# a-ludi/dentist

Hardware: AMD Instinct MI355X
Metric: gap-bases closed/sec (higher is better)
Workload: dtype u8

## Files before the change

### dentist_amd/csrc/dh_tjoin.h

```cpp
#ifndef DH_TJOIN_H
#define DH_TJOIN_H
#include <stdint.h>

#if defined(__HIPCC__)
#define TJ_HD __host__ __device__ __forceinline__
#else
#define TJ_HD inline
#endif

#define TJ_SLOT_BITS 14
#define TJ_SLOTS (1 << TJ_SLOT_BITS)
#define TJ_CAP 8192
#define TJ_THREADS 1024
#define TJ_RUN (TJ_THREADS / 64)
#define TJ_QBATCH 4
#define TJ_MAXK 16
#define TJ_EMPTY (~0ull)

#define DH_ST_TJ_HITCAP 0x80
#define DH_ST_TJ_OVERFLOW 0x100

TJ_HD uint32_t tj_home(uint32_t canon) { return (canon * 0x9E3779B1u) >> (32 - TJ_SLOT_BITS); }
TJ_HD uint64_t tj_slot(uint32_t canon, uint32_t ori, uint32_t idx) { return ((uint64_t)canon << 32) | (ori << 31) | idx; }

template <class Claim>
TJ_HD void tj_insert(uint64_t *tab, uint64_t v, Claim claim)
{
    uint32_t h = tj_home((uint32_t)(v >> 32));
    while (!claim(tab + h, v)) h = (h + 1) & (TJ_SLOTS - 1);
}

template <class F>
TJ_HD void tj_walk(const uint64_t *tab, uint32_t canon, F f)
{
    for (uint32_t h = tj_home(canon);; h = (h + 1) & (TJ_SLOTS - 1)) {
        const uint64_t s = tab[h];
        if (s == TJ_EMPTY) return;
        if ((uint32_t)(s >> 32) == canon) f((uint32_t)s);
    }
}

struct TjMatch {
    int32_t fwd, rev;
    uint32_t emit;
};
TJ_HD TjMatch tj_match(const uint64_t *tab, uint32_t canon, uint32_t bori, bool pal, int32_t tcap, int32_t strands)
{
    int32_t runf = 0, runr = 0;
    tj_walk(tab, canon, [&](uint32_t lo) {
        const bool same = (lo >> 31) == bori;
        runf += (same || pal) ? 1 : 0;
        runr += (!same || pal) ? 1 : 0;
    });
    TjMatch m;
    m.emit = ((runf > 0 && runf <= tcap && (strands & 1)) ? 1u : 0u) | ((runr > 0 && runr <= tcap && (strands & 2)) ? 2u : 0u);
    m.fwd = (m.emit & 1u) ? runf : 0;
    m.rev = (m.emit & 2u) ? runr : 0;
    return m;
}

#ifndef DH_TJOIN_SLOT_CODE_ONLY
#include "dh_device.h"
#include "dh_join.h"

struct TjView {
    const uint32_t *gent;
    int32_t ngroups;
    const int4 *units;
    int32_t nunits;
    int32_t read0;
    uint64_t *segtab;
    uint64_t *hits;
    int64_t hits_cap;
    unsigned long long *cursor;
    uint32_t *queue;
    int32_t *status;
};

extern "C" {
void dhk_tj_group_offsets(hipStream_t st, const uint32_t *dir, int32_t ngroups, int32_t k, int32_t shift, int64_t nb,
                          uint32_t *gent);
void dhk_tjoin(hipStream_t st, DbView B, IndexView ix, DhOpts o, TjView t, int32_t ncu);
}
#endif
#endif
```

### dentist_amd/csrc/dh_tjoin.hip

```cpp
#include <hip/hip_runtime.h>
#include <stdint.h>
#include <stdio.h>
#include <stdlib.h>

#include <algorithm>

#include "dh_kmer.h"
#include "dh_tjoin.h"

#define LANES 64
#define HIT_QBITS 24

#ifdef DH_TJ_PROF
__device__ unsigned long long g_tj_prof[4];
#define TP(i) if (tid == 0) { const unsigned long long t_ = wall_clock64(); atomicAdd(&g_tj_prof[i], t_ - tp_); tp_ = t_; }
#define TP_BEGIN unsigned long long tp_ = wall_clock64();
extern "C" void dhk_tj_prof_dump()
{
    unsigned long long h[4];
    (void)hipMemcpyFromSymbol(h, HIP_SYMBOL(g_tj_prof), sizeof(h));
    if (h[3])
        fprintf(stderr, "[tj prof] k_tjoin, %llu units: table build %.1f roll + probe %.1f write %.1f us per unit and block\n", h[3],
                h[0] / 100.0 / h[3], h[1] / 100.0 / h[3], h[2] / 100.0 / h[3]);
    unsigned long long z[4] = {0};
    (void)hipMemcpyToSymbol(HIP_SYMBOL(g_tj_prof), z, sizeof(z));
}
#else
#define TP(i)
#define TP_BEGIN
#endif

__global__ void __launch_bounds__(256)
k_tj_group_offsets(const uint32_t *__restrict__ dir, int32_t ngroups, int32_t k, int32_t shift, int64_t nb, uint32_t *__restrict__ gent)
{
    const int32_t g = blockIdx.x * blockDim.x + threadIdx.x;
    if (g > ngroups) return;
    int64_t b = (int64_t)(((uint64_t)g << (2 * k)) >> shift);
    b = b < nb ? b : nb;
    gent[g] = dir[b - 1];
}

static __device__ __forceinline__ uint32_t tj_pack8(uint64_t w)
{
    uint64_t x = __builtin_bswap64(w) & 0x0303030303030303ull;
    x = (x | (x >> 6)) & 0x000F000F000F000Full;
    x = (x | (x >> 12)) & 0x000000FF000000FFull;
    return (uint32_t)((x | (x >> 24)) & 0xFFFFull);
}

template <bool WRITE>
static __device__ uint32_t tj_read(const DbView &B, const IndexView &ix, const DhOpts &o, const KmerSampler &smp, const uint64_t *tab,
                                   int32_t r, int lane, uint32_t g0, uint64_t *__restrict__ out, uint32_t limit, uint32_t *cur)
{
    constexpr int PER = 8, STEP = LANES * PER;
    constexpr uint64_t BAD = 0xFCFCFCFCFCFCFCFCull;
    const int64_t bo = B.off[r];
    const int32_t blen = (int32_t)(B.off[r + 1] - bo);
    const uint8_t *b = B.bases + bo;
    const int k = o.k;
    const int32_t npos = blen - k + 1;
    const uint32_t kmask = k >= 16 ? 0xFFFFFFFFu : ((1u << (2 * k)) - 1u);
    const uint32_t kbits = (1u << k) - 1u;
    uint32_t cnt = 0;
    uint64_t n0 = 0, n1 = 0, n2 = 0, nm = 0;
    auto fetch = [&](int32_t q0) {
        if (q0 < npos) {
            n0 = load8(b + q0);
            n1 = load8(b + q0 + 8);
            n2 = load8(b + q0 + 16);
            if (B.mask_bits) nm = load8(B.mask_bits + ((bo + q0) >> 3)) >> ((bo + q0) & 7);
        }
    };
    fetch(lane * PER);
    for (int32_t base = 0; base < npos; base += STEP) {
        const int32_t q0 = base + lane * PER;
        const uint64_t w0 = n0, w1 = n1, w2 = n2;
        const uint32_t mbits = (uint32_t)nm;
        fetch(q0 + STEP);
        if (q0 >= npos) continue;
        uint32_t nbits = 0;
        if ((w0 | w1 | w2) & BAD) {
            for (int i = 0; i < 8; i++) {
                nbits |= (((w0 >> (8 * i)) & 0xFC) ? 1u : 0u) << i;
                nbits |= (((w1 >> (8 * i)) & 0xFC) ? 1u : 0u) << (8 + i);
                nbits |= (((w2 >> (8 * i)) & 0xFC) ? 1u : 0u) << (16 + i);
            }
        }
        const uint64_t P = ((uint64_t)tj_pack8(w0) << 32) | ((uint64_t)tj_pack8(w1) << 16) | (uint64_t)tj_pack8(w2);
        uint64_t R = __brevll(~P);
        R = (((R >> 1) & 0x5555555555555555ull) | ((R & 0x5555555555555555ull) << 1)) >> 16;
#pragma unroll
        for (int j = 0; j < PER; j++) {
            const int32_t q = q0 + j;
            const uint32_t km = (uint32_t)(P >> (48 - 2 * k - 2 * j)) & kmask;
            const uint32_t rc = (uint32_t)(R >> (2 * j)) & kmask;
            const uint32_t canon = km < rc ? km : rc;
            const bool em = q < npos && !(((nbits | mbits) >> j) & kbits) && kmer_sampled((uint64_t)canon, smp);
            if (!em) continue;
            const uint32_t bori = km != canon ? 1u : 0u;
            const bool pal = km == rc;
            const TjMatch m = tj_match(tab, canon, bori, pal, o.tcap, o.strands);
            if (!WRITE)
                cnt += (uint32_t)(m.fwd + m.rev);
            else if (m.emit) {
                tj_walk(tab, canon, [&](uint32_t lo) {
                    const bool same = (lo >> 31) == bori;
                    const int64_t gv = (int64_t)(ix.ent[g0 + (lo & 0x7FFFFFFFu)].y & ((1ull << 40) - 1));
                    for (int32_t strand = 0; strand < 2; strand++) {
                        if (!(m.emit & (1u << strand)) || !(strand ? (!same || pal) : (same || pal))) continue;
                        const int32_t qs = strand ? blen - k - q : q;
                        const int64_t D = gv + ix.sepv - qs;
                        const uint32_t slot = atomicAdd(cur, 1u);
                        if (slot < limit) out[slot] = ((uint64_t)strand << 63) | ((uint64_t)D << HIT_QBITS) | (uint32_t)qs;
                        cnt++;
                    }
                });
            }
        }
    }
    return cnt;
}

__global__ void __launch_bounds__(TJ_THREADS, 1)
k_tjoin(DbView B, IndexView ix, DhOpts o, TjView t)
{
    __shared__ uint64_t tab[TJ_SLOTS];
    __shared__ uint32_t s_cnt[TJ_RUN], s_cur[TJ_RUN];
    __shared__ unsigned long long s_base;
    __shared__ int32_t s_work, s_ok;
    const int tid = threadIdx.x, lane = tid & (LANES - 1), wv = tid / LANES;
    const KmerSampler smp = kmer_sampler(o.kmer_mod, o.k);
    const uint64_t kmask = (1ull << (2 * o.k)) - 1;
    int32_t have = -1;
    uint32_t g0 = 0;
    TP_BEGIN
    for (;;) {
        __syncthreads();
        if (tid == 0) s_work = (int32_t)atomicAdd(t.queue, (uint32_t)TJ_QBATCH);
        __syncthreads();
        const int32_t u0 = s_work;
        if (u0 >= t.nunits) break;
#pragma unroll 1
        for (int32_t u = u0; u < min(u0 + TJ_QBATCH, t.nunits); u++) {
            const int4 un = t.units[u];
            if (un.x != have) {
                have = un.x;
                uint32_t g1 = 0;
                g0 = 0;
                if ((uint32_t)un.x < (uint32_t)t.ngroups) {
                    g0 = t.gent[un.x];
                    g1 = t.gent[un.x + 1];
                }
                if (g1 - g0 > (uint32_t)TJ_CAP || g1 > (uint32_t)ix.n || g1 < g0) {
                    if (tid == 0) atomicOr(t.status, DH_ST_TJ_OVERFLOW);
                    g1 = g0;
                }
                for (int32_t i = tid; i < TJ_SLOTS; i += TJ_THREADS) tab[i] = TJ_EMPTY;
                __syncthreads();
                for (uint32_t e = g0 + tid; e < g1; e += TJ_THREADS) {
                    const uint64_t x = ix.ent[e].x;
                    tj_insert(tab, tj_slot((uint32_t)(x & kmask), (uint32_t)(x >> 63), e - g0), [](uint64_t *p, uint64_t v) {
                        return atomicCAS((unsigned long long *)p, (unsigned long long)TJ_EMPTY, (unsigned long long)v) == TJ_EMPTY;
                    });
                }
                __syncthreads();
                TP(0)
            }
            const int32_t r = un.y + wv;
            const bool mine = r < un.z;
            uint32_t c = mine ? tj_read<false>(B, ix, o, smp, tab, r, lane, g0, nullptr, 0u, nullptr) : 0u;
            for (int off = LANES / 2; off > 0; off >>= 1) c += __shfl_xor(c, off, LANES);
            if (lane == 0) {
                s_cnt[wv] = c;
                s_cur[wv] = 0;
            }
            __syncthreads();
            if (tid == 0) {
                unsigned long long total = 0;
                for (int i = 0; i < TJ_RUN; i++) total += s_cnt[i];
                const unsigned long long base = total ? atomicAdd(t.cursor, total) : 0ull;
                const bool ok = base + total <= (unsigned long long)t.hits_cap;
                if (!ok) atomicOr(t.status, DH_ST_TJ_HITCAP);
                s_base = base;
                s_ok = ok ? 1 : 0;
            }
            __syncthreads();
            TP(1)
            if (mine && s_ok) {
                unsigned long long first = s_base;
                for (int i = 0; i < wv; i++) first += s_cnt[i];
                if (c >= (1u << 24) || first >= (1ull << 40)) {
                    if (lane == 0) atomicOr(t.status, DH_ST_TJ_OVERFLOW);
                } else {
                    if (c) tj_read<true>(B, ix, o, smp, tab, r, lane, g0, t.hits + first, c, &s_cur[wv]);
                    if (lane == 0) t.segtab[r - t.read0] = (first << 24) | c;
                }
            }
            __syncthreads();
            TP(2)
#ifdef DH_TJ_PROF
            if (tid == 0) atomicAdd(&g_tj_prof[3], 1ull);
#endif
        }
    }
}

extern "C" void dhk_tj_group_offsets(hipStream_t st, const uint32_t *dir, int32_t ngroups, int32_t k, int32_t shift, int64_t nb,
                                     uint32_t *gent)
{
    hipLaunchKernelGGL(k_tj_group_offsets, dim3((unsigned)((ngroups + 1 + 255) / 256)), dim3(256), 0, st, dir, ngroups, k, shift, nb, gent);
}

extern "C" void dhk_tjoin(hipStream_t st, DbView B, IndexView ix, DhOpts o, TjView t, int32_t ncu)
{
    if (t.nunits <= 0) return;
    const int32_t batches = (t.nunits + TJ_QBATCH - 1) / TJ_QBATCH;
    hipLaunchKernelGGL(k_tjoin, dim3((unsigned)std::min(batches, std::max(1, ncu))), dim3(TJ_THREADS), 0, st, B, ix, o, t);
#ifdef DH_TJ_PROF
    if (getenv("DH_TRACE")) {
        (void)hipStreamSynchronize(st);
        dhk_tj_prof_dump();
    }
#endif
}
```

Measured before the change: 2.515 million.

## Stash matching k-mer positions in LDS to skip full re-scan in write pass

During the count pass, each wave records in a per-wave LDS stash the read positions whose k-mer produced hits. The write pass then recomputes only those k-mers from two 8-byte loads and emits hits, instead of re-rolling and re-probing the whole read. Reads that are too long or overflow the stash fall back to the original full second pass, and an env var forces the old two-pass path. This adds LDS usage, which might stay within one-block-per-CU occupancy, plus an extra atomic per matching position during counting.

```diff
diff --git a/dentist_amd/csrc/dh_tjoin.h b/dentist_amd/csrc/dh_tjoin.h
--- a/dentist_amd/csrc/dh_tjoin.h
+++ b/dentist_amd/csrc/dh_tjoin.h
@@ -15,6 +15,8 @@
 #define TJ_RUN (TJ_THREADS / 64)
 #define TJ_QBATCH 4
 #define TJ_MAXK 16
+#define TJ_STASH 1008
+#define TJ_STASH_POSBITS 16
 #define TJ_EMPTY (~0ull)
 
 #define DH_ST_TJ_HITCAP 0x80
@@ -59,6 +61,44 @@
     return m;
 }
 
+TJ_HD uint32_t tj_pack8(uint64_t w)
+{
+    uint64_t x = __builtin_bswap64(w) & 0x0303030303030303ull;
+    x = (x | (x >> 6)) & 0x000F000F000F000Full;
+    x = (x | (x >> 12)) & 0x000000FF000000FFull;
+    return (uint32_t)((x | (x >> 24)) & 0xFFFFull);
+}
+
+TJ_HD uint32_t tj_brev32(uint32_t x)
+{
+#if defined(__HIP_DEVICE_COMPILE__)
+    return __brev(x);
+#else
+    x = ((x >> 1) & 0x55555555u) | ((x & 0x55555555u) << 1);
+    x = ((x >> 2) & 0x33333333u) | ((x & 0x33333333u) << 2);
+    x = ((x >> 4) & 0x0F0F0F0Fu) | ((x & 0x0F0F0F0Fu) << 4);
+    return __builtin_bswap32(x);
+#endif
+}
+
+struct TjKmer {
+    uint32_t canon, bori;
+    bool pal;
+};
+TJ_HD TjKmer tj_kmer_at(uint64_t w0, uint64_t w1, int k)
+{
+    const uint32_t km = ((tj_pack8(w0) << 16) | tj_pack8(w1)) >> (32 - 2 * k);
+    uint32_t rc = tj_brev32(~km);
+    rc = (((rc >> 1) & 0x55555555u) | ((rc & 0x55555555u) << 1)) >> (32 - 2 * k);
+    TjKmer r;
+    r.canon = km < rc ? km : rc;
+    r.bori = km != r.canon ? 1u : 0u;
+    r.pal = km == rc;
+    return r;
+}
+
+TJ_HD bool tj_stash_fits(int32_t npos) { return npos <= (1 << TJ_STASH_POSBITS); }
+
 #ifndef DH_TJOIN_SLOT_CODE_ONLY
 #include "dh_device.h"
 #include "dh_join.h"
diff --git a/dentist_amd/csrc/dh_tjoin.hip b/dentist_amd/csrc/dh_tjoin.hip
--- a/dentist_amd/csrc/dh_tjoin.hip
+++ b/dentist_amd/csrc/dh_tjoin.hip
@@ -40,17 +40,29 @@
     gent[g] = dir[b - 1];
 }
 
-static __device__ __forceinline__ uint32_t tj_pack8(uint64_t w)
-{
-    uint64_t x = __builtin_bswap64(w) & 0x0303030303030303ull;
-    x = (x | (x >> 6)) & 0x000F000F000F000Full;
-    x = (x | (x >> 12)) & 0x000000FF000000FFull;
-    return (uint32_t)((x | (x >> 24)) & 0xFFFFull);
-}
-
-template <bool WRITE>
+enum { TJ_COUNT = 0, TJ_COUNT_STASH = 1, TJ_WRITE = 2 };
+
+static __device__ __forceinline__ void tj_emit(const IndexView &ix, const uint64_t *tab, uint32_t canon, uint32_t bori, bool pal,
+                                               uint32_t emit, int32_t q, int32_t blen, int k, uint32_t g0,
+                                               uint64_t *__restrict__ out, uint32_t limit, uint32_t *cur)
+{
+    tj_walk(tab, canon, [&](uint32_t lo) {
+        const bool same = (lo >> 31) == bori;
+        const int64_t gv = (int64_t)(ix.ent[g0 + (lo & 0x7FFFFFFFu)].y & ((1ull << 40) - 1));
+        for (int32_t strand = 0; strand < 2; strand++) {
+            if (!(emit & (1u << strand)) || !(strand ? (!same || pal) : (same || pal))) continue;
+            const int32_t qs = strand ? blen - k - q : q;
+            const int64_t D = gv + ix.sepv - qs;
+            const uint32_t slot = atomicAdd(cur, 1u);
+            if (slot < limit) out[slot] = ((uint64_t)strand << 63) | ((uint64_t)D << HIT_QBITS) | (uint32_t)qs;
+        }
+    });
+}
+
+template <int MODE>
 static __device__ uint32_t tj_read(const DbView &B, const IndexView &ix, const DhOpts &o, const KmerSampler &smp, const uint64_t *tab,
-                                   int32_t r, int lane, uint32_t g0, uint64_t *__restrict__ out, uint32_t limit, uint32_t *cur)
+                                   int32_t r, int lane, uint32_t g0, uint64_t *__restrict__ out, uint32_t limit, uint32_t *cur,
+                                   uint16_t *stash, uint32_t *stn)
 {
     constexpr int PER = 8, STEP = LANES * PER;
     constexpr uint64_t BAD = 0xFCFCFCFCFCFCFCFCull;
@@ -100,32 +112,43 @@
             const uint32_t bori = km != canon ? 1u : 0u;
             const bool pal = km == rc;
             const TjMatch m = tj_match(tab, canon, bori, pal, o.tcap, o.strands);
-            if (!WRITE)
-                cnt += (uint32_t)(m.fwd + m.rev);
-            else if (m.emit) {
-                tj_walk(tab, canon, [&](uint32_t lo) {
-                    const bool same = (lo >> 31) == bori;
-                    const int64_t gv = (int64_t)(ix.ent[g0 + (lo & 0x7FFFFFFFu)].y & ((1ull << 40) - 1));
-                    for (int32_t strand = 0; strand < 2; strand++) {
-                        if (!(m.emit & (1u << strand)) || !(strand ? (!same || pal) : (same || pal))) continue;
-                        const int32_t qs = strand ? blen - k - q : q;
-                        const int64_t D = gv + ix.sepv - qs;
-                        const uint32_t slot = atomicAdd(cur, 1u);
-                        if (slot < limit) out[slot] = ((uint64_t)strand << 63) | ((uint64_t)D << HIT_QBITS) | (uint32_t)qs;
-                        cnt++;
-                    }
-                });
+            if (MODE == TJ_WRITE) {
+                if (m.emit) tj_emit(ix, tab, canon, bori, pal, m.emit, q, blen, k, g0, out, limit, cur);
+                continue;
+            }
+            cnt += (uint32_t)(m.fwd + m.rev);
+            if (MODE == TJ_COUNT_STASH && m.emit) {
+                const uint32_t slot = atomicAdd(stn, 1u);
+                if (slot < (uint32_t)TJ_STASH) stash[slot] = (uint16_t)q;
             }
         }
     }
     return cnt;
 }
 
+static __device__ void tj_write_stashed(const DbView &B, const IndexView &ix, const DhOpts &o, const uint64_t *tab, int32_t r, int lane,
+                                        uint32_t g0, uint64_t *__restrict__ out, uint32_t limit, uint32_t *cur,
+                                        const uint16_t *stash, uint32_t n)
+{
+    const int64_t bo = B.off[r];
+    const int32_t blen = (int32_t)(B.off[r + 1] - bo);
+    const uint8_t *b = B.bases + bo;
+    for (uint32_t i = (uint32_t)lane; i < n; i += LANES) {
+        const int32_t q = (int32_t)stash[i];
+        const TjKmer km = tj_kmer_at(load8(b + q), load8(b + q + 8), o.k);
+        const TjMatch m = tj_match(tab, km.canon, km.bori, km.pal, o.tcap, o.strands);
+        tj_emit(ix, tab, km.canon, km.bori, km.pal, m.emit, q, blen, o.k, g0, out, limit, cur);
+    }
+}
+
+static_assert(TJ_STASH <= (1 << 16) && TJ_SLOTS * 8 + TJ_RUN * (TJ_STASH * 2 + 12) + 16 <= 160 * 1024, "table and stash share a CU's LDS");
+
 __global__ void __launch_bounds__(TJ_THREADS, 1)
-k_tjoin(DbView B, IndexView ix, DhOpts o, TjView t)
+k_tjoin(DbView B, IndexView ix, DhOpts o, TjView t, int32_t two_pass)
 {
     __shared__ uint64_t tab[TJ_SLOTS];
-    __shared__ uint32_t s_cnt[TJ_RUN], s_cur[TJ_RUN];
+    __shared__ uint16_t s_stash[TJ_RUN][TJ_STASH];
+    __shared__ uint32_t s_cnt[TJ_RUN], s_cur[TJ_RUN], s_stn[TJ_RUN];
     __shared__ unsigned long long s_base;
     __shared__ int32_t s_work, s_ok;
     const int tid = threadIdx.x, lane = tid & (LANES - 1), wv = tid / LANES;
@@ -168,7 +191,12 @@
             }
             const int32_t r = un.y + wv;
             const bool mine = r < un.z;
-            uint32_t c = mine ? tj_read<false>(B, ix, o, smp, tab, r, lane, g0, nullptr, 0u, nullptr) : 0u;
+            const bool stashing = mine && !two_pass && tj_stash_fits((int32_t)(B.off[r + 1] - B.off[r]) - o.k + 1);
+            if (lane == 0) s_stn[wv] = 0;
+            __builtin_amdgcn_wave_barrier();
+            uint32_t c = !mine      ? 0u
+                         : stashing ? tj_read<TJ_COUNT_STASH>(B, ix, o, smp, tab, r, lane, g0, nullptr, 0u, nullptr, s_stash[wv], &s_stn[wv])
+                                    : tj_read<TJ_COUNT>(B, ix, o, smp, tab, r, lane, g0, nullptr, 0u, nullptr, nullptr, nullptr);
             for (int off = LANES / 2; off > 0; off >>= 1) c += __shfl_xor(c, off, LANES);
             if (lane == 0) {
                 s_cnt[wv] = c;
@@ -192,7 +220,11 @@
                 if (c >= (1u << 24) || first >= (1ull << 40)) {
                     if (lane == 0) atomicOr(t.status, DH_ST_TJ_OVERFLOW);
                 } else {
-                    if (c) tj_read<true>(B, ix, o, smp, tab, r, lane, g0, t.hits + first, c, &s_cur[wv]);
+                    const uint32_t ns = s_stn[wv];
+                    if (c && stashing && ns <= (uint32_t)TJ_STASH)
+                        tj_write_stashed(B, ix, o, tab, r, lane, g0, t.hits + first, c, &s_cur[wv], s_stash[wv], ns);
+                    else if (c)
+                        tj_read<TJ_WRITE>(B, ix, o, smp, tab, r, lane, g0, t.hits + first, c, &s_cur[wv], nullptr, nullptr);
                     if (lane == 0) t.segtab[r - t.read0] = (first << 24) | c;
                 }
             }
@@ -215,7 +247,8 @@
 {
     if (t.nunits <= 0) return;
     const int32_t batches = (t.nunits + TJ_QBATCH - 1) / TJ_QBATCH;
-    hipLaunchKernelGGL(k_tjoin, dim3((unsigned)std::min(batches, std::max(1, ncu))), dim3(TJ_THREADS), 0, st, B, ix, o, t);
+    const int32_t two_pass = getenv("DH_TJOIN_TWO_PASS") ? 1 : 0;
+    hipLaunchKernelGGL(k_tjoin, dim3((unsigned)std::min(batches, std::max(1, ncu))), dim3(TJ_THREADS), 0, st, B, ix, o, t, two_pass);
 #ifdef DH_TJ_PROF
     if (getenv("DH_TRACE")) {
         (void)hipStreamSynchronize(st);
```

Measured after the change: 2.524 million, median of 6. No clear change (+0.4%).
